# amirhajibabaei/AutoForce

Measured on AMD Instinct MI355X. Metric: MD-step atoms*steps/sec (SGPR predict: NL + descriptors + K_nm + E/F/stress + covloss); `value`: a Langevin MD loop on the device, every step from the forces of the one before (sgpr_md_run; --steps dependent steps between two fences); `value_resident_frames`: steps over independent frames resident i, higher is better.
Workload: dtype f64

## Files before the change

### autoforce_amd/csrc/api.hip

```cpp
#include <math.h>
#include <stdarg.h>
#include <stdio.h>
#include <stdlib.h>
#include <string.h>

#include <algorithm>
#include <atomic>
#include <numeric>
#include <type_traits>

#include <dlfcn.h>
#include <unistd.h>
#include <rccl/rccl.h>

#include "../../include/sgpr_hip.h"
#include "sgpr_internal.h"
#include "nl_grid.inc"
#include <cmath>
#include <limits>

static thread_local char g_err[512] = "";
static int fail(int code, const char *fmt, ...)
{
    va_list ap;
// ... 2407 lines not shown
        return fail(SGPR_E_UNSUPPORTED, "sgpr_md_run: the filter (sgpr_md_filter) runs in the gather form of the fused last kernel only");
    if (nx && nx->mode == 2 && h->md.run.meta.on) {
        const MdState &m = h->md;
        if (!(fuse && gather))
            return fail(SGPR_E_UNSUPPORTED, "sgpr_md_run: the bias (sgpr_md_meta) runs in the gather form of the fused last kernel only: the scatter form "
                                            "and sharded frames take the host loop around calculate()");
        const long long n = nx->md.t_index;
        MetaQl ql = m.run.meta.ql;
        if (m.run.meta.nql) {
            if ((long long)m.run.meta.nql * h->maxnn > META_QL_MAXT)
                return fail(SGPR_E_UNSUPPORTED, "sgpr_md_run: the bias has %d qlvar component(s) and the neighbour list holds up to %d entries per atom; together at "
                                                "most %d (the host loop around calculate() serves longer lists)", m.run.meta.nql, h->maxnn, META_QL_MAXT);
            ql.nn = h->d_nn.p; ql.nbr_j = h->d_nbr_j.p; ql.nbr_code = h->d_nbr_shift.p; ql.cell = cell_dev; ql.maxnn = h->maxnn;
        }
        if (m.run.meta.nql && m.run.meta.merge) {
            const long long want = m.run.meta_slot(n) / m.run.meta.merge;
            for (long long &j = h->md.run.meta.enq; j < want; j++) {
                hipLaunchKernelGGL(md_meta_merge_kernel, dim3(1), dim3(256), 0, st, m.run.meta.par.D, m.run.meta.merge, (int)j, (const double *)m.meta.centre.p,
                                   (const int *)m.meta.key.p, m.meta_tab(want), (const int *)nx->md.halt, (int)step);
                stamp(h, "md_meta_merge", st);
            }
            hipLaunchKernelGGL(md_meta_merged_ql_kernel, dim3((N + 255) / 256), dim3(256), 0, st, N, m.run.meta.par, ql, nx->md.x_cur, (const unsigned char *)m.meta.sel.p,
                               m.meta.centre.p, m.meta.key.p, m.meta.rows.p, (int)m.run.meta_slot(n), n % m.run.meta.pace == 0 ? (int)m.run.meta_slot(n) : -1,
                               h->d_F.p + 3 * (size_t)N, h->d_Epart.p, h->d_virpart.p, h->virpart_len, m.meta_tab(want), (const int *)nx->md.halt, (int)step);
        } else if (m.run.meta.nql) {
            hipLaunchKernelGGL(md_meta_ql_kernel, dim3((N + 255) / 256), dim3(256), 0, st, N, m.run.meta.par, ql, nx->md.x_cur, (const unsigned char *)m.meta.sel.p,
                               m.meta.centre.p, m.meta.key.p, m.meta.rows.p, (int)m.run.meta_slot(n), n % m.run.meta.pace == 0 ? (int)m.run.meta_slot(n) : -1,
                               h->d_F.p + 3 * (size_t)N, h->d_Epart.p, h->d_virpart.p, h->virpart_len, (const int *)nx->md.halt, (int)step);
        } else if (m.run.meta.merge) {
            const long long want = m.run.meta_slot(n) / m.run.meta.merge;
            for (long long &j = h->md.run.meta.enq; j < want; j++) {
                hipLaunchKernelGGL(md_meta_merge_kernel, dim3(1), dim3(256), 0, st, m.run.meta.par.D, m.run.meta.merge, (int)j, (const double *)m.meta.centre.p,
                                   (const int *)m.meta.key.p, m.meta_tab(want), (const int *)nx->md.halt, (int)step);
                stamp(h, "md_meta_merge", st);
            }
            hipLaunchKernelGGL(md_meta_merged_kernel, dim3((N + 255) / 256), dim3(256), 0, st, N, m.run.meta.par, nx->md.x_cur, (const unsigned char *)m.meta.sel.p,
                               m.meta.centre.p, m.meta.key.p, m.meta.rows.p, (int)m.run.meta_slot(n), n % m.run.meta.pace == 0 ? (int)m.run.meta_slot(n) : -1,
                               h->d_F.p + 3 * (size_t)N, h->d_Epart.p, h->d_virpart.p, h->virpart_len, m.meta_tab(want), (const int *)nx->md.halt, (int)step);
        } else
            hipLaunchKernelGGL(md_meta_kernel, dim3((N + 255) / 256), dim3(256), 0, st, N, m.run.meta.par, nx->md.x_cur, (const unsigned char *)m.meta.sel.p,
                               m.meta.centre.p, m.meta.key.p, m.meta.rows.p, (int)m.run.meta_slot(n), n % m.run.meta.pace == 0 ? (int)m.run.meta_slot(n) : -1,
                               h->d_F.p + 3 * (size_t)N, h->d_Epart.p, h->d_virpart.p, h->virpart_len, (const int *)nx->md.halt, (int)step);
        stamp(h, "md_meta", st);
    }
    const bool xp = !gather && (px || shard_next);
    const size_t xlen = peer_xlen(N, h->world);
    if (xp && h->d_xpacked.n < xlen + 1 && h->d_xpacked.alloc(xlen + 1)) return fail(SGPR_E_NODEVICE, "hipMalloc failed (exchange buffer)");
    launch_finalize(h, gather && predict, predict ? (fused3 ? 4 * (int)h->t_knm.n : h->epart_len) : 0, predict ? h->virpart_len : 0, beta, h->mean_energy,
                    xp ? h->d_xpacked.p : packed_dev, st, nullptr, fuse ? nx : nullptr, step, xp);
    h->reduce_done = false;
    if (shard_next) {
        stamp(h, "finalize", st);
        ShardSrc src;
        src.base = h->d_xpacked.p; src.n = 1; src.stride = 0; src.ctl = nullptr; src.cmax = (int)peer_cmax(N, h->world);
        if (px) {
            int parity = 0;
            if (h->peer.world != h->world || h->peer.rank != h->rank)
                return fail(SGPR_E_INVALID, "the bound sharding (rank %d of %d) differs from the exchange's (rank %d of %d)",
                            h->rank, h->world, h->peer.rank, h->peer.world);
            const int *halt = nx->mode == 2 ? nx->md.halt : nullptr;
            const int re = peer_exchange(h, h->d_xpacked.p, xlen, st, &parity, halt, (int)step);
            if (re) return re;
            src = peer_src(h->peer, parity);
            src.cmax = (int)peer_cmax(N, h->world);
            stamp(h, "exchange", st);
        }
        launch_finalize(h, false, 0, 0, beta, h->mean_energy, packed_dev, st, nullptr, nx, step, false, &src);
        h->reduce_done = true;
    }
    if (fuse || shard_next) {
        h->pre_valid = true; h->pre_pos = nx->pos_next; h->pre_cell = nx->cell_next ? nx->cell_next : cell_dev; h->pre_step = step + 1;
    }
    stamp(h, shard_next ? "sum_bin_next" : fuse ? "finalize_bin_next" : "finalize", st);
    return SGPR_OK;
}

static int run_checked(sgpr_model *h, const double *pos_dev, const double *cell_dev, double *packed_dev,
                       hipStream_t st)
{
    if (h->maxnn == 0) {
        const int rc_ = ensure_nl(h, 64);
        if (rc_) return rc_;
    }
    if (h->bin_cap == 0) {
        const int rc_ = ensure_bins(h, 64);
        if (rc_) return rc_;
    }
    if (h->world == 1 && h->gather_ok && h->t_stride == 0) {
        const int rc_ = ensure_rev(h, 27 * h->bin_cap);
        if (rc_) return rc_;
    }
    for (int attempt = 0; attempt < 12; attempt++) {
        HIPCHK(hipMemsetAsync(h->d_stat.p, 0, 4 * sizeof(int), st));
        HIPCHK(hipMemsetAsync(h->d_bin_count.p, 0, 2 * SGPR_BIN_INTS * sizeof(int), st));
        h->pre_valid = false;
        const int rc_ = enqueue_step(h, pos_dev, cell_dev, packed_dev, st, nullptr, true);
        if (rc_) return rc_;
        HIPCHK(hipStreamSynchronize(st));
        HIPCHK(hipGetLastError());
        int stat[4] = {0, 0, 0, 0};
        HIPCHK(hipMemcpy(stat, h->d_stat.p, 4 * sizeof(int), hipMemcpyDeviceToHost));
        if (stat[3] == 2) return fail(SGPR_E_INVALID, "the cell vector of a periodic direction is zero");
        if (stat[3] == 4) {
            h->gemm_fused = false;
            fprintf(stderr, "[sgpr] the fused GEMM launch timed out waiting for its K_nm tiles: continuing with separate launches\n");
            continue;
        }
        if (stat[3] == 3) return fail(SGPR_E_OVERFLOW, "a pair force beyond 1024 eV/A left the fixed-point range of the sharded reverse pass");
        if (stat[3])
            return fail(SGPR_E_OVERFLOW, "an atom lies more than 127 periodic images away from a neighbour (or > 32767 "
                        "cells from the origin): wrap the positions into the cell");
        if (stat[1] > h->bin_cap) {
            int cap = h->bin_cap;
            while (cap < stat[1] + stat[1] / 4) cap *= 2;
            const int rc2 = ensure_bins(h, cap);
            if (rc2) return rc2;
            if (h->world == 1 && h->gather_ok) {
                const int rc3 = ensure_rev(h, std::max(h->t_stride, 27 * cap));
                if (rc3) return rc3;
            }
            continue;
        }
        if (stat[2] > h->t_stride && h->world == 1 && h->gather_ok) {
            if (stat[2] == 0x7fffffff || (double)stat[2] * std::max(h->N, 1) > 2e9) h->gather_ok = false;
            else {
                const int rc3 = ensure_rev(h, stat[2]);
                if (rc3) return rc3;
            }
            continue;
        }
        if (stat[0] <= h->maxnn) {
            h->nn_max_seen = stat[0];
            HIPCHK(hipMemset(h->d_stat.p, 0, 4 * sizeof(int)));
            h->lists_valid = true;
            return SGPR_OK;
        }
        h->lists_valid = false;
        if (stat[0] > 100000) return fail(SGPR_E_OVERFLOW, "neighbour count %d is unreasonable", stat[0]);
        const int rc2 = ensure_nl(h, rup(stat[0] + stat[0] / 8 + 4, 8));
        if (rc2) return rc2;
    }
    return fail(SGPR_E_OVERFLOW, "neighbour capacity kept overflowing");
}

static int reduce_packed(sgpr_model *h, double *packed_dev, hipStream_t st)
{
    if (h->reduce_done) { h->reduce_done = false; return SGPR_OK; }
    if (peer_on(h)) {
        if (h->world == 1) return SGPR_OK;
        if (h->peer.world != h->world || h->peer.rank != h->rank)
            return fail(SGPR_E_INVALID, "the bound sharding (rank %d of %d) differs from the exchange's (rank %d of %d)",
                        h->rank, h->world, h->peer.rank, h->peer.world);
        int parity = 0;
        const int re = peer_exchange(h, h->d_xpacked.p, peer_xlen(h->N, h->world), st, &parity);
        if (re) return re;
        ShardSrc src = peer_src(h->peer, parity);
        src.cmax = (int)peer_cmax(h->N, h->world);
        hipLaunchKernelGGL(peer_sum_xp_kernel, dim3(std::min(256, (4 * std::max(h->N, 1) + 11 + 255) / 256)), dim3(256), 0, st,
                           src, h->N, packed_dev, (const int *)h->peer.ctl.p, (const int *)(h->d_perm.p + h->N));
        return SGPR_OK;
    }
    if (!h->comm) return SGPR_OK;
    if (h->world == 1) return SGPR_OK;
    if (h->comm_world != h->world || h->comm_rank != h->rank)
        return fail(SGPR_E_INVALID, "the bound sharding (rank %d of %d) differs from the communicator's (rank %d of %d)",
                    h->rank, h->world, h->comm_rank, h->comm_world);
    const ncclResult_t r = g_rccl.AllReduce(packed_dev, packed_dev, (size_t)sgpr_packed_len(h->N), ncclDouble, ncclSum, h->comm, st);
    if (r != ncclSuccess) return fail(SGPR_E_NODEVICE, "ncclAllReduce: %s", g_rccl.GetErrorString(r));
    return SGPR_OK;
}

extern "C" int sgpr_comm_unique_id(void *id_out)
{
    if (!id_out) return fail(SGPR_E_INVALID, "sgpr_comm_unique_id: bad arguments");
    if (const int rl = rccl_load()) return rl;
    ncclUniqueId id;
    const ncclResult_t r = g_rccl.GetUniqueId(&id);
    if (r != ncclSuccess) return fail(SGPR_E_NODEVICE, "ncclGetUniqueId: %s", g_rccl.GetErrorString(r));
    static_assert(sizeof(id) == SGPR_COMM_ID_BYTES, "ncclUniqueId size");
    memcpy(id_out, &id, sizeof(id));
    return SGPR_OK;
}

extern "C" int sgpr_comm_init(sgpr_model *h, const void *id_in, int rank, int world)
{
    if (!h || !id_in || world < 1 || rank < 0 || rank >= world) return fail(SGPR_E_INVALID, "sgpr_comm_init: bad arguments");
    if (const int rl = rccl_load()) return rl;
    HIPCHK(hipSetDevice(h->device));
    if (h->comm) { (void)g_rccl.CommDestroy(h->comm); h->comm = nullptr; }
    ncclUniqueId id;
    memcpy(&id, id_in, sizeof(id));
    const ncclResult_t r = g_rccl.CommInitRank(&h->comm, world, id, rank);
    if (r != ncclSuccess) { h->comm = nullptr; return fail(SGPR_E_NODEVICE, "ncclCommInitRank: %s", g_rccl.GetErrorString(r)); }
    h->comm_rank = rank; h->comm_world = world;
    drop_graph(h);
    return SGPR_OK;
}

extern "C" int sgpr_comm_destroy(sgpr_model *h)
{
    if (!h) return fail(SGPR_E_INVALID, "sgpr_comm_destroy: bad arguments");
// ... 501 lines not shown
```

### autoforce_amd/csrc/descriptor.hip

```cpp
#include "sgpr_internal.h"
#include "gemm_tile.inc"

__constant__ HarmCoef c_hc;

void upload_harm_coef(const HarmCoef &hc) { (void)hipMemcpyToSymbol(HIP_SYMBOL(c_hc), &hc, sizeof(HarmCoef)); }

#define SQRT2 1.4142135623730951
typedef double v4d __attribute__((ext_vector_type(4)));

__device__ __forceinline__ void wave_sync()
{
    __builtin_amdgcn_fence(__ATOMIC_RELEASE, "wavefront");
    __builtin_amdgcn_wave_barrier();
    __builtin_amdgcn_fence(__ATOMIC_ACQUIRE, "wavefront");
}

__device__ __forceinline__ double uniform(double v)
{
    const int lo = __builtin_amdgcn_readfirstlane(__double2loint(v));
    const int hi = __builtin_amdgcn_readfirstlane(__double2hiint(v));
    return __hiloint2double(hi, lo);
}

template <typename T>
// ... 395 lines not shown
#pragma unroll
                    for (int k = 0; k < SPL; k++) {
                        const int slot = lane + 64 * k;
                        if (SPL * 64 == NSLOT || slot < NSLOT)
                            acc[q][k] += fl[tt * N1 + slot / LL] * Yl[tt * LLP + slot % LL];
                    }
                }
                beg = end;
            }
        } else {
#pragma unroll 4
            for (int tt = 0; tt < cnt; tt++) {
                const int s = __builtin_amdgcn_readfirstlane(sl[tt]);
#pragma unroll
                for (int k = 0; k < SPL; k++) {
                    const int slot = lane + 64 * k;
                    if (SPL * 64 == NSLOT || slot < NSLOT) {
                        const double v = fl[tt * N1 + slot / LL] * Yl[tt * LLP + slot % LL];
#pragma unroll
                        for (int q = 0; q < ST; q++)
                            if (s == q) acc[q][k] += v;
                    }
                }
            }
        }
    }
    wave_sync();
#pragma unroll
    for (int s = 0; s < ST; s++)
#pragma unroll
        for (int k = 0; k < SPL; k++) {
            const int slot = lane + 64 * k;
            if (SPL * 64 == NSLOT || slot < NSLOT) {
                cl[s * NSLOT + slot] = acc[s][k];
                if (a.C && s < a.S) a.C[(size_t)ia * a.CS + s * NSLOT + slot] = acc[s][k];
            }
        }
    wave_sync();
    double nrm2 = 0.0;
    constexpr int L1 = LMAX + 1;
    constexpr int UMAX = ST * N1;
    constexpr int MAXP = ((UMAX * (UMAX + 1)) / 2 + 63) / 64;
    const int npair = a.Dc / L1;
    double pv[MAXP][L1];
#pragma unroll
    for (int k = 0; k < MAXP; k++) {
        const int pr = lane + 64 * k;
#pragma unroll
        for (int l = 0; l < L1; l++) pv[k][l] = 0.0;
        if (pr < npair) {
            const PackEntry p0 = a.pack[pr * L1];
            const double *cu = cl + (p0.u / N1) * NSLOT + (p0.u % N1) * LL;
            const double *cv = cl + (p0.v / N1) * NSLOT + (p0.v % N1) * LL;
#pragma unroll
            for (int l = 0; l < L1; l++) {
                double sacc = 0.0;
#pragma unroll
                for (int mm = 0; mm < 2 * l + 1; mm++) sacc += cu[l * l + mm] * cv[l * l + mm];
                pv[k][l] = sacc * a.pack[pr * L1 + l].coef;
                nrm2 += pv[k][l] * pv[k][l];
            }
        }
    }
    nrm2 = wave_sum(nrm2);
    const double nrm = sqrt(nrm2);
    const double inv = nn > 0 ? 1.0 / (nrm + SGPR_EPS) : 0.0;
#pragma unroll
    for (int k = 0; k < MAXP; k++) {
        const int pr = lane + 64 * k;
        if (pr < npair) {
#pragma unroll
            for (int l = 0; l < L1; l++) a.Pn[(size_t)ia * a.Dpad + pr * L1 + l] = pv[k][l] * inv;
        }
    }
    for (int e = a.Dc + lane; e < a.Dpad; e += 64) a.Pn[(size_t)ia * a.Dpad + e] = 0.0;
    if (lane == 0) {
        a.norm[ia] = nn > 0 ? nrm : 0.0;
        if (a.shear) a.shear[ia] = shear ? 1 : 0;
    }
}

#define NL_SORT_MAX 256
#ifndef NL_STEPS
#define NL_STEPS 4
#endif

struct NlArgs {
    const NlGrid *grid;
    const int *bin_of, *kslot, *bin_count;
    int cap;
    const BinRec *b_rec;
    const BinAux *b_aux;
    int *nn, *nn_local, *nn_raw, *nbr_j, *nbr_shift, *aux;
    unsigned short *T;
    int t_stride;
    int *stat;
    const int *flag;
    double rc_list;
    int *ncand, *cand_j, *cand_code, *cidx;
    unsigned long long *hm;
    int hmw;
};

#ifdef SGPR_PHASE_STAMPS
#define PHASE_STAMP(K) if (a.stamps && lane == 0) a.stamps[(size_t)ia * 8 + (K)] = (long long)__builtin_amdgcn_s_memtime()
#else
#define PHASE_STAMP(K)
#endif

template <int LMAX, int NMAX, int ST>
struct FwdLds {
    using WL = WaveLds<LMAX, NMAX>;
    static constexpr int CH = WL::CHS;
    static constexpr int BINL = NL_SORT_MAX + NL_SORT_MAX / 2, HIT0 = BINL + 2 * 64;
    static constexpr int NLV = HIT0 + 4 * CH;
    static constexpr int FWV = CH * WL::N1 + CH * WL::RS;
    static constexpr int P4V = ST * WL::NSLOT + 16;
    static constexpr int RA = (NLV > FWV ? (NLV > P4V ? NLV : P4V) : (FWV > P4V ? FWV : P4V));
    static constexpr int PW = RA;
};

template <int LMAX, int NMAX, int ST>
__global__ __launch_bounds__(256, 4) void nl_fwd_kernel(DescArgs a, NlArgs n)
{
    using WL = WaveLds<LMAX, NMAX>;
    using FL = FwdLds<LMAX, NMAX, ST>;
    constexpr int N1 = WL::N1, LL = WL::LL, NSLOT = WL::NSLOT, CH = WL::CHS;
    constexpr int UC = ST * N1, CBS = (UC + 15) / 16, RBL = (LL + 15) / 16;
    extern __shared__ double smem[];
    const int wave = __builtin_amdgcn_readfirstlane(threadIdx.x >> 6), lane = threadIdx.x & 63;
    const int ia = xcd_quad((int)blockIdx.x, (int)gridDim.x, a.xq) * 4 + wave;
    if (ia >= a.N) return;
    const int i = a.first + ia * a.stride;
    double *wbase = smem + (size_t)wave * FL::PW;
    double *RA = wbase;
    unsigned long long *keys = (unsigned long long *)RA;
    int *hq = (int *)(RA + NL_SORT_MAX);
    int4 *binl = (int4 *)(RA + FL::BINL);
    double *hit0 = RA + FL::HIT0;
    double *fl = RA;
    double *Yl = fl + CH * N1;
    double *cl = RA;

    PHASE_STAMP(0);
    const int cap = n.cap, maxnn = a.maxnn;
    double h[9];
#pragma unroll
    for (int k = 0; k < 9; k++) h[k] = a.cell[k];
    const double xi = uniform(a.pos[3 * (size_t)i]), yi = uniform(a.pos[3 * (size_t)i + 1]), zi = uniform(a.pos[3 * (size_t)i + 2]);
    const int ki = __builtin_amdgcn_readfirstlane(n.kslot[i]);
    const bool ghost = ki < 0;
    const unsigned long long lt = lane == 0 ? 0ull : (~0ull >> (64 - lane));
    const bool rebuild = __builtin_amdgcn_readfirstlane(*n.flag) != 0;
    int ncand = 0;
    int j_first = 0, cd_first = 0;
    if (rebuild) {
        const NlGrid g = *n.grid;
        const int bi = __builtin_amdgcn_readfirstlane(n.bin_of[i]);
        int wi0 = 0, wi1 = 0, wi2 = 0;
        if (ki >= 0 && ki < cap) {
            const BinAux own = n.b_aux[(size_t)bi * cap + ki];
            wi0 = own.w0; wi1 = own.w1; wi2 = own.w2;
        }
        auto fdiv = [](int q, float inv) { return (int)(((float)q + 0.5f) * inv); };
        const float i_n2 = 1.0f / (float)g.nb[2], i_n1 = 1.0f / (float)g.nb[1];
        const int bq = fdiv(bi, i_n2);
        const int b2 = bi - bq * g.nb[2];
        const int b0 = fdiv(bq, i_n1);
        const int b1 = bq - b0 * g.nb[1];
        const int w0 = 2 * g.rng[0] + 1, w1 = 2 * g.rng[1] + 1, w2 = 2 * g.rng[2] + 1;
        const float i_w2 = 1.0f / (float)w2, i_w1 = 1.0f / (float)w1;
        const double r_n0 = 1.0 / g.nb[0], r_n1 = 1.0 / g.nb[1], r_n2 = 1.0 / g.nb[2];
        const int nbox = w0 * w1 * w2;
        const bool t_ok = n.T != nullptr && (long long)nbox * cap <= (long long)n.t_stride && cap <= 4096 && maxnn <= 65535 &&
                          ki < cap && !ghost;
        if (n.T != nullptr && !t_ok && ki < cap && !ghost && lane == 0)
            atomicMax(&n.stat[2], cap <= 4096 && maxnn <= 65535 ? nbox * cap : 0x7fffffff);
        const int grp = lane >> 4, s16 = lane & 15;
        const double rl2 = n.rc_list * n.rc_list;
        int base = 0;
        auto consume = [&](bool valid, const BinRec &rec, const BinAux &ax, int code, int q, int k) {
            bool hit = false;
            int f0 = 0, f1 = 0, f2 = 0;
            if (valid) {
                f0 = (int)(int8_t)(code & 0xff) - ax.w0 + wi0;
                f1 = (int)(int8_t)((code >> 8) & 0xff) - ax.w1 + wi1;
                f2 = (int)(int8_t)((code >> 16) & 0xff) - ax.w2 + wi2;
                const double dx = rec.x - xi + (f0 * h[0] + f1 * h[3] + f2 * h[6]);
                const double dy = rec.y - yi + (f0 * h[1] + f1 * h[4] + f2 * h[7]);
                const double dz = rec.z - zi + (f0 * h[2] + f1 * h[5] + f2 * h[8]);
                hit = dx * dx + dy * dy + dz * dz < rl2 && !(rec.idx == i && f0 == 0 && f1 == 0 && f2 == 0);
            }
            const unsigned long long m = __ballot(hit);
            if (hit) {
                const int slot = base + __popcll(m & lt);
                const int j = rec.idx, sj = ax.slot;
                const unsigned img = (unsigned)((f0 + 128) & 0xff) << 16 | (unsigned)((f1 + 128) & 0xff) << 8 |
                                     (unsigned)((f2 + 128) & 0xff);
                const unsigned long long key = ((unsigned long long)(unsigned)j << 40) | ((unsigned long long)img << 16) |
                                               ((unsigned long long)(unsigned)sj << 12) | (unsigned)(slot & 0xfff);
                if (max(max(abs(f0), abs(f1)), abs(f2)) > 127) atomicMax(&n.stat[3], 1);
                if (slot < NL_SORT_MAX) {
                    keys[slot] = key;
                    hq[slot] = (q << 12) | k;
                } else if (slot < maxnn) {
                    const size_t e = (size_t)i * maxnn + slot;
                    n.cand_j[e] = j;
                    n.cand_code[e] = (f0 & 0xff) | ((f1 & 0xff) << 8) | ((f2 & 0xff) << 16) | (sj << 24);
                    n.aux[e] = 0;
                    if (t_ok) {
                        n.aux[e] = q * cap + k;
                        n.T[(size_t)j * n.t_stride + (size_t)(nbox - 1 - q) * cap + ki] = (unsigned short)slot;
                    }
                }
            }
            base += __popcll(m);
        };
        constexpr int STEPS = NL_STEPS;
        double tb[3];
#pragma unroll
        for (int k = 0; k < 3; k++) {
            const double fk = xi * g.inv[k] + yi * g.inv[3 + k] + zi * g.inv[6 + k];
            const double uk = (fk - floor(fk)) * g.nb[k] - (k == 0 ? b0 : k == 1 ? b1 : b2);
            tb[k] = g.rng[k] > 0 ? fmin(fmax(uk, 0.0), 1.0) : 0.0;
        }
        const double rl2_skip = rl2 * (1.0 + 1e-9);
        for (int q0 = 0; q0 < (ghost ? 0 : nbox); q0 += 64) {
            int nbin_l = 0, code_l = 0, cnt_l = 0;
            bool keep = false;
            {
                const int q = q0 + lane;
                if (q < nbox) {
                    const int qa = fdiv(q, i_w2), qb = fdiv(qa, i_w1);
                    const int o2 = q - qa * w2 - g.rng[2], o1 = qa - qb * w1 - g.rng[1], o0 = qb - g.rng[0];
                    const int t0 = b0 + o0, t1 = b1 + o1, t2 = b2 + o2;
                    const int c0 = (int)floor((double)t0 * r_n0 + 1e-9), c1 = (int)floor((double)t1 * r_n1 + 1e-9),
                              c2 = (int)floor((double)t2 * r_n2 + 1e-9);
                    nbin_l = ((t0 - c0 * g.nb[0]) * g.nb[1] + (t1 - c1 * g.nb[1])) * g.nb[2] + (t2 - c2 * g.nb[2]);
                    code_l = (c0 & 0xff) | ((c1 & 0xff) << 8) | ((c2 & 0xff) << 16);
                    cnt_l = min(n.bin_count[(size_t)nbin_l * SGPR_BIN_STRIDE], cap);
                    const double g0 = (o0 > 0 ? o0 - tb[0] : o0 < 0 ? tb[0] - o0 - 1.0 : 0.0) * g.w[0];
                    const double g1 = (o1 > 0 ? o1 - tb[1] : o1 < 0 ? tb[1] - o1 - 1.0 : 0.0) * g.w[1];
                    const double g2 = (o2 > 0 ? o2 - tb[2] : o2 < 0 ? tb[2] - o2 - 1.0 : 0.0) * g.w[2];
                    const double gm = fmax(g0, fmax(g1, g2));
                    const double lb2 = g.ortho ? g0 * g0 + g1 * g1 + g2 * g2 : gm * gm;
                    keep = cnt_l > 0 && lb2 < rl2_skip;
                }
            }
            const unsigned long long km = __ballot(keep);
            const int nlist = __popcll(km);
            wave_sync();
            if (keep) binl[__popcll(km & lt)] = make_int4(nbin_l, code_l, cnt_l, q0 + lane);
            wave_sync();
            const int nsteps = (nlist + 3) >> 2;
            for (int u0 = 0; u0 < nsteps; u0 += STEPS) {
                int nbin[STEPS], code[STEPS], cnt[STEPS], qq[STEPS], cmax = 0;
#pragma unroll
                for (int u = 0; u < STEPS; u++) {
                    const int e = 4 * (u0 + u) + grp;
                    const int4 bb = binl[e < nlist ? e : 0];
                    nbin[u] = bb.x; code[u] = bb.y; qq[u] = bb.w;
                    cnt[u] = e < nlist ? bb.z : 0;
                    cmax = max(cmax, cnt[u]);
                }
                for (int s0 = 0; __any(s0 < cmax); s0 += 16) {
                    BinRec rec[STEPS];
                    BinAux ax[STEPS];
#pragma unroll
                    for (int u = 0; u < STEPS; u++) {
                        const size_t e = (size_t)nbin[u] * cap + (s0 + s16 < cnt[u] ? s0 + s16 : 0);
                        rec[u] = n.b_rec[e];
                        ax[u] = n.b_aux[e];
                    }
#pragma unroll
                    for (int u = 0; u < STEPS; u++)
                        if (__any(s0 + s16 < cnt[u])) consume(s0 + s16 < cnt[u], rec[u], ax[u], code[u], qq[u], s0 + s16);
                }
            }
        }
        PHASE_STAMP(1);
        const int ns = min(base, NL_SORT_MAX);
        wave_sync();
        if (ns <= 64) {
            unsigned long long key = lane < ns ? keys[lane] : ~0ull;
#pragma unroll
            for (int k2s = 2; k2s <= 64; k2s <<= 1)
#pragma unroll
                for (int j2 = k2s >> 1; j2 > 0; j2 >>= 1) {
                    const unsigned lo = __shfl_xor((unsigned)key, j2, 64), hi = __shfl_xor((unsigned)(key >> 32), j2, 64);
                    const unsigned long long other = ((unsigned long long)hi << 32) | lo;
                    const bool lower = (lane & j2) == 0, up = (lane & k2s) == 0;
                    const bool take_min = lower == up;
                    key = take_min ? (other < key ? other : key) : (other > key ? other : key);
                }
            wave_sync();
            if (lane < ns) keys[lane] = key;
        } else {
            int np2 = 1;
            while (np2 < ns) np2 <<= 1;
            for (int t = ns + lane; t < np2; t += 64) keys[t] = ~0ull;
            wave_sync();
            for (int k2s = 2; k2s <= np2; k2s <<= 1)
                for (int j2 = k2s >> 1; j2 > 0; j2 >>= 1) {
                    for (int t = lane; t < np2; t += 64) {
                        const int p = t ^ j2;
                        if (p > t) {
                            const unsigned long long a0 = keys[t], a1 = keys[p];
                            const bool up = (t & k2s) == 0;
                            if ((a0 > a1) == up) { keys[t] = a1; keys[p] = a0; }
                        }
                    }
                    wave_sync();
                }
        }
        wave_sync();
        ncand = base < maxnn ? base : maxnn;
        for (int c = lane; c < ns && c < maxnn; c += 64) {
            const unsigned long long key = keys[c];
            const unsigned img = (unsigned)(key >> 16) & 0xffffffu;
            const int f0 = (int)((img >> 16) & 0xff) - 128, f1 = (int)((img >> 8) & 0xff) - 128, f2 = (int)(img & 0xff) - 128,
                      sj = (int)(key >> 12) & 0xf, j = (int)(key >> 40);
            const size_t e = (size_t)i * maxnn + c;
            n.cand_j[e] = j;
            n.cand_code[e] = (f0 & 0xff) | ((f1 & 0xff) << 8) | ((f2 & 0xff) << 16) | (sj << 24);
            int hs = 0;
            if (t_ok) {
                const int hv = hq[(int)key & 0xfff];
                const int qv = hv >> 12, kk = hv & 0xfff;
                hs = qv * cap + kk;
                n.T[(size_t)j * n.t_stride + (size_t)(nbox - 1 - qv) * cap + ki] = (unsigned short)c;
            }
            n.aux[e] = hs;
        }
        if (lane == 0) {
            n.ncand[i] = ncand;
            n.nn_raw[ia] = base;
        }
        if (ncand > NL_SORT_MAX) __threadfence();
        PHASE_STAMP(2);
    } else {
        const int nc_v = n.ncand[i];
        if (lane < maxnn) {
            const size_t e = (size_t)i * maxnn + lane;
            j_first = n.cand_j[e];
            cd_first = n.cand_code[e];
        }
        ncand = __builtin_amdgcn_readfirstlane(nc_v);
        if (lane == 0) n.nn_raw[ia] = ncand;
    }
    const double rc2_lo = a.rc * a.rc * (1.0 - 1e-14), rc2_hi = a.rc * a.rc * (1.0 + 1e-14);
    int nn = 0;
    bool near = false;
    for (int c0 = 0; c0 < ncand; c0 += 64) {
        const int c = c0 + lane;
        bool hit = false;
        int j = 0, cd = 0;
        double r0 = 1.0, r1 = 0.0, r2 = 0.0;
        if (c < ncand) {
            if (rebuild && c < NL_SORT_MAX) {
                const unsigned long long key = keys[c];
// ... 830 lines not shown
```

### autoforce_amd/csrc/nl_grid.inc

```
#pragma once

__device__ __forceinline__ double det3d(const double *h)
{
    return h[0] * (h[4] * h[8] - h[5] * h[7]) - h[1] * (h[3] * h[8] - h[5] * h[6]) + h[2] * (h[3] * h[7] - h[4] * h[6]);
}

__device__ inline void nl_make_grid(const double *cell, const int *pbc, double rc, NlGrid &g, int *stat)
{
    double h[9];
    for (int k = 0; k < 9; k++) h[k] = cell[k];
    {
        int zero[3], nz = 0;
        for (int k = 0; k < 3; k++) {
            zero[k] = h[3 * k] * h[3 * k] + h[3 * k + 1] * h[3 * k + 1] + h[3 * k + 2] * h[3 * k + 2] < 1e-24;
            nz += zero[k];
            if (zero[k] && pbc[k] && stat) atomicMax(&stat[3], 2);
        }
        if (nz > 0 && nz < 3) {
            for (int k = 0; k < 3; k++) {
                if (!zero[k] || pbc[k]) continue;
                const double *p = h + 3 * ((k + 1) % 3), *q = h + 3 * ((k + 2) % 3);
                double v[3];
                if (!zero[(k + 1) % 3] && !zero[(k + 2) % 3]) {
                    v[0] = p[1] * q[2] - p[2] * q[1]; v[1] = p[2] * q[0] - p[0] * q[2]; v[2] = p[0] * q[1] - p[1] * q[0];
                } else {
                    const double *w = zero[(k + 1) % 3] ? q : p;
                    const int a = fabs(w[0]) <= fabs(w[1]) && fabs(w[0]) <= fabs(w[2]) ? 0 : (fabs(w[1]) <= fabs(w[2]) ? 1 : 2);
                    double e[3] = {0.0, 0.0, 0.0};
                    e[a] = 1.0;
                    v[0] = w[1] * e[2] - w[2] * e[1]; v[1] = w[2] * e[0] - w[0] * e[2]; v[2] = w[0] * e[1] - w[1] * e[0];
                }
                const double nv = sqrt(v[0] * v[0] + v[1] * v[1] + v[2] * v[2]);
                if (nv > 1e-12) {
                    h[3 * k] = v[0] / nv; h[3 * k + 1] = v[1] / nv; h[3 * k + 2] = v[2] / nv;
                    zero[k] = 0;
                }
            }
        }
    }
    const double dt = det3d(h);
    if (fabs(dt) > 1e-12) {
        const double *p = h, *q = h + 3, *r = h + 6;
        const double bc[3] = {q[1] * r[2] - q[2] * r[1], q[2] * r[0] - q[0] * r[2], q[0] * r[1] - q[1] * r[0]};
        const double ca[3] = {r[1] * p[2] - r[2] * p[1], r[2] * p[0] - r[0] * p[2], r[0] * p[1] - r[1] * p[0]};
        const double ab[3] = {p[1] * q[2] - p[2] * q[1], p[2] * q[0] - p[0] * q[2], p[0] * q[1] - p[1] * q[0]};
        for (int k = 0; k < 3; k++) {
            g.inv[3 * k + 0] = bc[k] / dt;
            g.inv[3 * k + 1] = ca[k] / dt;
            g.inv[3 * k + 2] = ab[k] / dt;
        }
        const double V = fabs(dt);
        const double hgt[3] = {V / sqrt(bc[0] * bc[0] + bc[1] * bc[1] + bc[2] * bc[2]),
                               V / sqrt(ca[0] * ca[0] + ca[1] * ca[1] + ca[2] * ca[2]),
                               V / sqrt(ab[0] * ab[0] + ab[1] * ab[1] + ab[2] * ab[2])};
        for (int k = 0; k < 3; k++) {
            if (pbc[k]) {
                int nb = (int)floor(hgt[k] / rc);
                nb = nb < 1 ? 1 : (nb > 16 ? 16 : nb);
                g.nb[k] = nb;
                g.rng[k] = (int)ceil(rc * nb / hgt[k]);
            } else {
                g.nb[k] = 1;
                g.rng[k] = 0;
            }
            g.w[k] = hgt[k] / g.nb[k];
        }
        const double d01 = bc[0] * ca[0] + bc[1] * ca[1] + bc[2] * ca[2], d02 = bc[0] * ab[0] + bc[1] * ab[1] + bc[2] * ab[2],
                     d12 = ca[0] * ab[0] + ca[1] * ab[1] + ca[2] * ab[2];
        const double n0 = bc[0] * bc[0] + bc[1] * bc[1] + bc[2] * bc[2], n1 = ca[0] * ca[0] + ca[1] * ca[1] + ca[2] * ca[2],
                     n2 = ab[0] * ab[0] + ab[1] * ab[1] + ab[2] * ab[2];
        g.ortho = (d01 * d01 < 1e-20 * n0 * n1 && d02 * d02 < 1e-20 * n0 * n2 && d12 * d12 < 1e-20 * n1 * n2) ? 1 : 0;
    } else {
        for (int k = 0; k < 9; k++) g.inv[k] = 0.0;
        for (int k = 0; k < 3; k++) { g.nb[k] = 1; g.rng[k] = 0; g.w[k] = 0.0; }
        g.ortho = 0;
    }
    g.nbins = g.nb[0] * g.nb[1] * g.nb[2];
}

__device__ __forceinline__ int nl_place_axis(const NlGrid &g, int k, int periodic, double X, double Y, double Z, int &w)
{
    double fr = X * g.inv[k] + Y * g.inv[3 + k] + Z * g.inv[6 + k];
    w = 0;
    if (!(periodic && (g.inv[k] != 0.0 || g.inv[3 + k] != 0.0 || g.inv[6 + k] != 0.0))) return 0;
    const double fl = floor(fr);
    w = (int)fl;
    fr -= fl;
    const int b = (int)(fr * g.nb[k]);
    return b >= g.nb[k] ? g.nb[k] - 1 : (b < 0 ? 0 : b);
}

__device__ __forceinline__ int nl_bin_index(const NlGrid &g, const int (&bidx)[3])
{
    return (bidx[0] * g.nb[1] + bidx[1]) * g.nb[2] + bidx[2];
}

__device__ __forceinline__ void nl_store_rec(BinRec *b_rec, BinAux *b_aux, int cap, int *stat, int bin, int k, double X, double Y, double Z,
                                             int idx, const int (&w)[3], int slot)
{
    if (max(max(abs(w[0]), abs(w[1])), abs(w[2])) > 32767) atomicMax(&stat[3], 1);
    if (k < cap) {
        const size_t e = (size_t)bin * cap + k;
        BinRec r;
        r.x = X; r.y = Y; r.z = Z; r.idx = idx; r.pad = 0;
        b_rec[e] = r;
        BinAux ax;
        ax.w0 = (short)w[0]; ax.w1 = (short)w[1]; ax.w2 = (short)w[2]; ax.slot = (short)slot;
        b_aux[e] = ax;
    } else
        atomicMax(&stat[1], k + 1);
}
```

### autoforce_amd/csrc/sgpr_internal.h

```cpp
#pragma once
#include <hip/hip_runtime.h>
#include <stdint.h>

#include <string>
#include <vector>

#define SGPR_MAX_S 16
#define SGPR_REV_WPW(S) ((S) > 8 ? 1 : 4)
#define SGPR_MAX_L 4
#define SGPR_MAX_N 4
#define SGPR_EPS 2.220446049250313e-16
#define SGPR_TINY_ANGLE 1e-2
#define SGPR_FIX_SCALE 70368744177664.0
#define SGPR_FIX_LIMIT 1024.0

struct HarmCoef {
    double y00;
    double al[SGPR_MAX_L + 1][SGPR_MAX_L + 1];
    double bl[SGPR_MAX_L + 1][SGPR_MAX_L + 1];
    double cl[SGPR_MAX_L + 1];
    double dl[SGPR_MAX_L + 1];
};

struct PackEntry {
// ... 32 lines not shown
    double h[9];
    double eta[9];
    double hinv[9];
    double bm1[9];
    double bp1inv[9];
    double aff_keep[9];
    double aff_reb[9];
    double thr2_keep, thr2_reb;
    double pad[15];
    NlGrid grid;
};
static_assert(sizeof(NptSlot) % 16 == 0, "slots of the ring stay aligned");

struct NptParams {
    double dt, c1, c2, K0;
    double pfact;
    double ext[6];
    double mask[9];
    double frac;
    double rc_list, rc_phys;
    int pbc[3];
};

#define META_MAXD 6
#define META_MAXC 4
#define META_TRIP 1024

struct MetaPar {
    int D, ncomp, wt, pad_;
    int kind[META_MAXC];
    int ia[META_MAXC];
    int ib[META_MAXC];
    double nsel[META_MAXC];
    double sigma[META_MAXD];
    double sigma5[META_MAXD];
    double w, gamma, norm;
};

#define META_QL_MAXL 12
#define META_QL_TINY_ANGLE 1e-2
#define META_QL_MAXT 256
struct MetaQl {
    const int *nn, *nbr_j, *nbr_code;
    const double *cell;
    int maxnn, pad_;
    int slot[META_MAXC];
    int nl[META_MAXC];
    double cut[META_MAXC];
    int dcomp[META_MAXD];
    int dl[META_MAXD];
};

enum { META_CTL_T = 0 , META_CTL_DONE = 1 , META_CTL_TPREV = 2 ,
       META_CTL_RUN = 3 , META_CTL_LEN = 4 };
struct MetaTab {
    double *centre;
    int *key;
    double *cnt;
    double *last;
    int *stamp;
    int *ctl;
    int ch, want;
};

struct RelaxParams {
    double fmax2;
    double dt0, maxstep, dtmax, finc, fdec, astart, fa;
    double nmin;
    double mask[9];
    double h0[9];
    double cf;
    int cell;
};

enum { RLX_DT = 0, RLX_A = 1, RLX_NSTEPS = 2, RLX_FRESH = 3, RLX_XC = 4 , RLX_VC = 13 ,
       RLX_ALPHA = 22, RLX_BETA = 23, RLX_CD = 24, RLX_LEN = 32 };
#define RLX_CELL 18
#define RLX_RING 9

struct NebCell { double h[9], hi[9]; int pbc[3]; };

#define SGPR_BIN_STRIDE 32
#define SGPR_BIN_INTS (4096 * SGPR_BIN_STRIDE)

struct BinRec { double x, y, z; int idx; int pad; };
struct BinAux { short w0, w1, w2, slot; };

struct NlScratch {
    NlGrid *grid;
    int *bin_of;
    int *kslot;
    int *bin_count;
    int cap;
    BinRec *b_rec;
    BinAux *b_aux;
    const int *slot;
    int *stat;
    int *nn_raw;
    int *aux;
    unsigned short *T;
    int t_stride;
    int *flag;
    int parity;
    int fslot, fclear;
    int force;
    double skin;
    double *pos0;
    double *cell0;
    int *ncand, *cand_j, *cand_code, *cidx;
    unsigned long long *hm;
    int hmw;
};

void launch_neighbor_bin(const NlParams &p, const int *perm, const double *pos_in, double *pos, const double *cell,
                         double rc, NlScratch s, double *zero_a, int n_zero_a, double *zero_b, int n_zero_b,
                         hipStream_t st);

struct DescParams {
    int lmax, nmax, S;
    int N;
    int Nall;
    int first, stride;
    int maxnn;
    int Dc, Dpad;
    int CS;
    double radii_v[SGPR_MAX_S];
    double rc;
    long long *stamps;
    int xq;
    int *stat;
};

int launch_list_forward(const DescParams &p, const NlScratch &nl, const double *pos, const double *cell,
                        const PackEntry *pack, int *nn , int *nn_local ,
                        int *nbr_j, int *nbr_shift, double *Pn , double *norm ,
                        double *C , int *shear ,
                        double *prec , hipStream_t st);

int launch_descriptor_forward_env(const DescParams &p, const int64_t *env_ptr, const int *env_slot,
                                  const double *env_r, const double *radii, const PackEntry *pack,
                                  double *Pn, double *norm, hipStream_t st);

struct RowsBatch {
    const double *aw;
    const double *pm;
    const int *cols;
    const int *col_slot;
    int ld, batch;
    size_t g_stride, f_stride, v_stride;
};

int launch_descriptor_backward(const DescParams &p, const double *pos, const double *cell,
                               const int *slot, const double *radii, const int *nn, const int *nbr_j,
                               const int *nbr_shift, const PackEntry *pack, const double *Pn,
                               const double *norm, const double *C, const int *shear,
                               const double *W , const double *prec ,
                               double *G , const int *aux, const unsigned short *T,
                               int t_stride, const int *cidx, const unsigned long long *hm, int hmw,
                               double *F ,
                               double *virial , hipStream_t st, const RowsBatch *rows = nullptr,
                               const struct GemmParams *cov = nullptr );

struct Rows16Params {
    const double *aw;
    const double *k;
    double eta;
// ... 81 lines not shown
```

Baseline: 51.11 million.

## Halve neighbour-list bin width and flatten candidate scan with prefix-sum indexing

Neighbour-list cells are now subdivided so each bin spans half the cutoff, giving 5x5x5 candidate boxes instead of 3x3x3. This shrinks the searched volume and the number of candidate pairs tested. The per-bin 16-lane group scan is replaced by a wave-wide prefix sum over bin populations plus a binary search, so every lane processes one candidate and lanes are no longer wasted on uneven bin counts. The initial bin capacity and reverse-table sizes are adjusted to match. In exchange the search adds shuffle scans, LDS binary searches and more boxes per atom, and the index arithmetic moves to float.

```diff
diff --git a/autoforce_amd/csrc/api.hip b/autoforce_amd/csrc/api.hip
--- a/autoforce_amd/csrc/api.hip
+++ b/autoforce_amd/csrc/api.hip
@@ -2513,12 +2513,15 @@
         const int rc_ = ensure_nl(h, 64);
         if (rc_) return rc_;
     }
+    const bool bulk = h->pbc[0] && h->pbc[1] && h->pbc[2];
+    int boxes = 1;
+    for (int k = 0; k < 3; k++) boxes *= h->pbc[k] ? 2 * SGPR_BIN_SUB + 1 : 1;
     if (h->bin_cap == 0) {
-        const int rc_ = ensure_bins(h, 64);
+        const int rc_ = ensure_bins(h, bulk ? 16 : 64);
         if (rc_) return rc_;
     }
     if (h->world == 1 && h->gather_ok && h->t_stride == 0) {
-        const int rc_ = ensure_rev(h, 27 * h->bin_cap);
+        const int rc_ = ensure_rev(h, boxes * h->bin_cap);
         if (rc_) return rc_;
     }
     for (int attempt = 0; attempt < 12; attempt++) {
@@ -2547,7 +2550,7 @@
             const int rc2 = ensure_bins(h, cap);
             if (rc2) return rc2;
             if (h->world == 1 && h->gather_ok) {
-                const int rc3 = ensure_rev(h, std::max(h->t_stride, 27 * cap));
+                const int rc3 = ensure_rev(h, std::max(h->t_stride, boxes * cap));
                 if (rc3) return rc3;
             }
             continue;
diff --git a/autoforce_amd/csrc/descriptor.hip b/autoforce_amd/csrc/descriptor.hip
--- a/autoforce_amd/csrc/descriptor.hip
+++ b/autoforce_amd/csrc/descriptor.hip
@@ -501,7 +501,7 @@
 
 #define NL_SORT_MAX 256
 #ifndef NL_STEPS
-#define NL_STEPS 4
+#define NL_STEPS 0
 #endif
 
 struct NlArgs {
@@ -589,13 +589,12 @@
         const int b1 = bq - b0 * g.nb[1];
         const int w0 = 2 * g.rng[0] + 1, w1 = 2 * g.rng[1] + 1, w2 = 2 * g.rng[2] + 1;
         const float i_w2 = 1.0f / (float)w2, i_w1 = 1.0f / (float)w1;
-        const double r_n0 = 1.0 / g.nb[0], r_n1 = 1.0 / g.nb[1], r_n2 = 1.0 / g.nb[2];
+        const float i_n0 = 1.0f / (float)g.nb[0];
         const int nbox = w0 * w1 * w2;
         const bool t_ok = n.T != nullptr && (long long)nbox * cap <= (long long)n.t_stride && cap <= 4096 && maxnn <= 65535 &&
                           ki < cap && !ghost;
         if (n.T != nullptr && !t_ok && ki < cap && !ghost && lane == 0)
             atomicMax(&n.stat[2], cap <= 4096 && maxnn <= 65535 ? nbox * cap : 0x7fffffff);
-        const int grp = lane >> 4, s16 = lane & 15;
         const double rl2 = n.rc_list * n.rc_list;
         int base = 0;
         auto consume = [&](bool valid, const BinRec &rec, const BinAux &ax, int code, int q, int k) {
@@ -635,7 +634,7 @@
             }
             base += __popcll(m);
         };
-        constexpr int STEPS = NL_STEPS;
+        constexpr int STEPS = NL_STEPS ? NL_STEPS : (ST == 1 ? 2 : 4);
         double tb[3];
 #pragma unroll
         for (int k = 0; k < 3; k++) {
@@ -644,57 +643,65 @@
             tb[k] = g.rng[k] > 0 ? fmin(fmax(uk, 0.0), 1.0) : 0.0;
         }
         const double rl2_skip = rl2 * (1.0 + 1e-9);
-        for (int q0 = 0; q0 < (ghost ? 0 : nbox); q0 += 64) {
-            int nbin_l = 0, code_l = 0, cnt_l = 0;
-            bool keep = false;
-            {
-                const int q = q0 + lane;
-                if (q < nbox) {
-                    const int qa = fdiv(q, i_w2), qb = fdiv(qa, i_w1);
-                    const int o2 = q - qa * w2 - g.rng[2], o1 = qa - qb * w1 - g.rng[1], o0 = qb - g.rng[0];
-                    const int t0 = b0 + o0, t1 = b1 + o1, t2 = b2 + o2;
-                    const int c0 = (int)floor((double)t0 * r_n0 + 1e-9), c1 = (int)floor((double)t1 * r_n1 + 1e-9),
-                              c2 = (int)floor((double)t2 * r_n2 + 1e-9);
-                    nbin_l = ((t0 - c0 * g.nb[0]) * g.nb[1] + (t1 - c1 * g.nb[1])) * g.nb[2] + (t2 - c2 * g.nb[2]);
-                    code_l = (c0 & 0xff) | ((c1 & 0xff) << 8) | ((c2 & 0xff) << 16);
-                    cnt_l = min(n.bin_count[(size_t)nbin_l * SGPR_BIN_STRIDE], cap);
-                    const double g0 = (o0 > 0 ? o0 - tb[0] : o0 < 0 ? tb[0] - o0 - 1.0 : 0.0) * g.w[0];
-                    const double g1 = (o1 > 0 ? o1 - tb[1] : o1 < 0 ? tb[1] - o1 - 1.0 : 0.0) * g.w[1];
-                    const double g2 = (o2 > 0 ? o2 - tb[2] : o2 < 0 ? tb[2] - o2 - 1.0 : 0.0) * g.w[2];
-                    const double gm = fmax(g0, fmax(g1, g2));
-                    const double lb2 = g.ortho ? g0 * g0 + g1 * g1 + g2 * g2 : gm * gm;
-                    keep = cnt_l > 0 && lb2 < rl2_skip;
-                }
-            }
-            const unsigned long long km = __ballot(keep);
-            const int nlist = __popcll(km);
+        static_assert(FL::HIT0 == FL::BINL + 2 * 64 && 4 * CH >= 2 * 64, "the second half of a chunk's bin list lies in the (idle) hit rows");
+        auto box = [&](int q, int &nbin_l, int &code_l) -> int {
+            nbin_l = 0; code_l = 0;
+            if (q >= nbox) return 0;
+            const int qa = fdiv(q, i_w2), qb = fdiv(qa, i_w1);
+            const int o2 = q - qa * w2 - g.rng[2], o1 = qa - qb * w1 - g.rng[1], o0 = qb - g.rng[0];
+            const int t0 = b0 + o0, t1 = b1 + o1, t2 = b2 + o2;
+            const int c0 = (int)floorf(((float)t0 + 0.5f) * i_n0), c1 = (int)floorf(((float)t1 + 0.5f) * i_n1),
+                      c2 = (int)floorf(((float)t2 + 0.5f) * i_n2);
+            nbin_l = ((t0 - c0 * g.nb[0]) * g.nb[1] + (t1 - c1 * g.nb[1])) * g.nb[2] + (t2 - c2 * g.nb[2]);
+            code_l = (c0 & 0xff) | ((c1 & 0xff) << 8) | ((c2 & 0xff) << 16);
+            const int cnt_l = min(n.bin_count[(size_t)nbin_l * SGPR_BIN_STRIDE], cap);
+            const double g0 = (o0 > 0 ? o0 - tb[0] : o0 < 0 ? tb[0] - o0 - 1.0 : 0.0) * g.w[0];
+            const double g1 = (o1 > 0 ? o1 - tb[1] : o1 < 0 ? tb[1] - o1 - 1.0 : 0.0) * g.w[1];
+            const double g2 = (o2 > 0 ? o2 - tb[2] : o2 < 0 ? tb[2] - o2 - 1.0 : 0.0) * g.w[2];
+            const double gm = fmax(g0, fmax(g1, g2));
+            const double lb2 = g.ortho ? g0 * g0 + g1 * g1 + g2 * g2 : gm * gm;
+            return lb2 < rl2_skip ? cnt_l : 0;
+        };
+        auto running = [&](int v) {
+#pragma unroll
+            for (int d = 1; d < 64; d <<= 1) {
+                const int t = __shfl_up(v, d, 64);
+                if (lane >= d) v += t;
+            }
+            return v;
+        };
+        for (int q0 = 0; q0 < (ghost ? 0 : nbox); q0 += 128) {
+            int nbin_a, code_a, nbin_b, code_b;
+            const int pop_a = box(q0 + lane, nbin_a, code_a), pop_b = box(q0 + 64 + lane, nbin_b, code_b);
+            const int end_a = running(pop_a);
+            const int tot_a = __builtin_amdgcn_readlane(end_a, 63);
+            const int end_b = tot_a + running(pop_b);
+            const int tot = __builtin_amdgcn_readlane(end_b, 63);
             wave_sync();
-            if (keep) binl[__popcll(km & lt)] = make_int4(nbin_l, code_l, cnt_l, q0 + lane);
+            binl[lane] = make_int4(nbin_a, code_a, end_a, end_a - pop_a);
+            binl[64 + lane] = make_int4(nbin_b, code_b, end_b, end_b - pop_b);
             wave_sync();
-            const int nsteps = (nlist + 3) >> 2;
-            for (int u0 = 0; u0 < nsteps; u0 += STEPS) {
-                int nbin[STEPS], code[STEPS], cnt[STEPS], qq[STEPS], cmax = 0;
+            for (int p0 = 0; p0 < tot; p0 += 64 * STEPS) {
+                int code[STEPS], qq[STEPS], ks[STEPS];
+                BinRec rec[STEPS];
+                BinAux ax[STEPS];
 #pragma unroll
                 for (int u = 0; u < STEPS; u++) {
-                    const int e = 4 * (u0 + u) + grp;
-                    const int4 bb = binl[e < nlist ? e : 0];
-                    nbin[u] = bb.x; code[u] = bb.y; qq[u] = bb.w;
-                    cnt[u] = e < nlist ? bb.z : 0;
-                    cmax = max(cmax, cnt[u]);
-                }
-                for (int s0 = 0; __any(s0 < cmax); s0 += 16) {
-                    BinRec rec[STEPS];
-                    BinAux ax[STEPS];
-#pragma unroll
-                    for (int u = 0; u < STEPS; u++) {
-                        const size_t e = (size_t)nbin[u] * cap + (s0 + s16 < cnt[u] ? s0 + s16 : 0);
-                        rec[u] = n.b_rec[e];
-                        ax[u] = n.b_aux[e];
-                    }
-#pragma unroll
-                    for (int u = 0; u < STEPS; u++)
-                        if (__any(s0 + s16 < cnt[u])) consume(s0 + s16 < cnt[u], rec[u], ax[u], code[u], qq[u], s0 + s16);
-                }
+                    if (p0 + 64 * u >= tot) continue;
+                    const int p = min(p0 + 64 * u + lane, tot - 1);
+                    int e = 0;
+#pragma unroll
+                    for (int st = 64; st > 0; st >>= 1)
+                        if (binl[e + st - 1].z <= p) e += st;
+                    const int4 bb = binl[e];
+                    code[u] = bb.y; qq[u] = q0 + e; ks[u] = p - bb.w;
+                    const size_t r = (size_t)bb.x * cap + ks[u];
+                    rec[u] = n.b_rec[r];
+                    ax[u] = n.b_aux[r];
+                }
+#pragma unroll
+                for (int u = 0; u < STEPS; u++)
+                    if (p0 + 64 * u < tot) consume(p0 + 64 * u + lane < tot, rec[u], ax[u], code[u], qq[u], ks[u]);
             }
         }
         PHASE_STAMP(1);
diff --git a/autoforce_amd/csrc/nl_grid.inc b/autoforce_amd/csrc/nl_grid.inc
--- a/autoforce_amd/csrc/nl_grid.inc
+++ b/autoforce_amd/csrc/nl_grid.inc
@@ -55,7 +55,7 @@
                                V / sqrt(ab[0] * ab[0] + ab[1] * ab[1] + ab[2] * ab[2])};
         for (int k = 0; k < 3; k++) {
             if (pbc[k]) {
-                int nb = (int)floor(hgt[k] / rc);
+                int nb = (int)floor(SGPR_BIN_SUB * hgt[k] / rc);
                 nb = nb < 1 ? 1 : (nb > 16 ? 16 : nb);
                 g.nb[k] = nb;
                 g.rng[k] = (int)ceil(rc * nb / hgt[k]);
diff --git a/autoforce_amd/csrc/sgpr_internal.h b/autoforce_amd/csrc/sgpr_internal.h
--- a/autoforce_amd/csrc/sgpr_internal.h
+++ b/autoforce_amd/csrc/sgpr_internal.h
@@ -138,6 +138,8 @@
 
 #define SGPR_BIN_STRIDE 32
 #define SGPR_BIN_INTS (4096 * SGPR_BIN_STRIDE)
+
+#define SGPR_BIN_SUB 2
 
 struct BinRec { double x, y, z; int idx; int pad; };
 struct BinAux { short w0, w1, w2, slot; };
```

After: 50.83 million, median of 2. No clear change (-0.5%).
